# sczhou/ProPainter

Hardware: NVIDIA B200
Metric: inpainted frames/sec at 432x240x80f (higher is better)
Workload: dtype f32 (TF32 tensor-core products, fp32 accumulate)

## Files before the change

### include/propainter_b200.h

```cpp
#ifndef PROPAINTER_B200_H
#define PROPAINTER_B200_H
#include <stddef.h>
#include <stdint.h>
#include <cuda_runtime_api.h>

#ifdef __cplusplus
extern "C" {
#endif

#define PP_ABI_VERSION 2
int pp_abi_version(void);
const char* pp_error_string(int code);

int pp_corr_build(const float* fmap, int D, const int* idx1, const int* idx2, int n_pairs, float* lvl0, int h, int w,
                  cudaStream_t stream);
int pp_corr_pool_pyramid(float* const* levels, long planes, int h, int w, cudaStream_t stream);
int pp_corr_lookup(const float* const* levels, const float* coords, float* out, long n_pairs, int h, int w,
                   cudaStream_t stream);
int pp_corr_lookup_ldg(const float* const* levels, const float* coords, float* out, long n_pairs, int h, int w,
                       cudaStream_t stream);
int pp_convex_upsample(const float* mask, int ld_mask, float mask_scale, const float* flow_lr, float* out, int n,
                       int h, int w, cudaStream_t stream);

size_t pp_img_prop_scan_workspace_bytes(int t, int H, int W);
// ... 1 lines not shown
                     float* out_frames, float* out_masks, void* workspace, size_t ws_bytes, int t, int H, int W,
                     int nearest, cudaStream_t stream);
int pp_prop_cond(const float* cur, int ld_cur, const float* prop, int ld_prop, const float* fprop,
                 const float* fcheck, const float* mcur, float* cond, int ld_cond, float* bb, int ld_bb, int h, int w,
                 int C, int first, cudaStream_t stream);
size_t pp_deform_align_workspace_bytes(int H, int W);
int pp_deform_align(const float* x, int ld_x, const float* o, int ld_o, const float* o_bias, const float* flow, float max_res,
                    const float* w_packed, const float* bias, float* out, int ld_out, int H, int W, int Cin, int Cout,
                    void* workspace, size_t ws_bytes, cudaStream_t stream);
#define PP_CONV_MAX_SEG 4
typedef struct PPConvSeg { const float* x; int ld; int C; } PPConvSeg;
typedef struct PPConvParams {
  PPConvSeg seg[PP_CONV_MAX_SEG];
  int nseg;
  int n, H, W, KH, KW;
  const float* w_packed;
  int Cout;
  const float* bias;
  const float* pre; int ld_pre;
  const float* res; int ld_res;
  float* out; int ld_out;
  int act; float slope; int post_relu; int round_tf32;
  int bn, tile_w, tile_m;
} PPConvParams;
int pp_conv2d_umma(const PPConvParams* prm, cudaStream_t stream);
int pp_conv2d_umma_plan(const PPConvParams* prm, int* tile_h, int* tile_w, int* bn, int* ctas, int* smem_bytes);
int pp_deform_gather(const float* x, int ld_x, const float* x2, int ld_x2, const float* o, int ld_o, const float* o_bias,
                     const float* flow, float max_res, float* cols, int n, int H, int W, int Cin, cudaStream_t stream);
int pp_flow_warp_fbcheck(const float* feat, int ld_f, const float* fprop, const float* fcheck, float* warped, int ld_w,
                         float* aux, int ld_a, int n, int h, int w, int C, int round_tf32, cudaStream_t stream);

int pp_gen_prep(const float* flows_f, const float* flows_b, const float* masks_in, const float* masks_upd, float* dsf,
                float* dsb, float* pmask, int lt, int H, int W, cudaStream_t stream);
int pp_window_mask(const float* pmask, int lt, int h, int w, int fh, int fw, int nwh, int nww, int* flags,
                   cudaStream_t stream);

typedef struct PPAttnParams {
  const float* qkv;
  const float* pool;
  const int* key_tok;
  const int* flags;
  float* out;
  int ld_qkv, ld_pool, ld_out;
  int t, NT, WN, NKO, NP, C;
  int kf_start, kf_step, nkf;
  float scale_log2;
} PPAttnParams;
int pp_sparse_window_attn(const PPAttnParams* prm, int n_windows, cudaStream_t stream);
int pp_sparse_window_attn_mma(const PPAttnParams* prm, int n_windows, cudaStream_t stream);
// ... 50 lines not shown
```

### propainter_b200/_lib.py

```python
import ctypes
import os

_HERE = os.path.dirname(os.path.abspath(__file__))
LIB_PATH = os.environ.get("PROPAINTER_B200_LIB") or os.path.join(_HERE, "libpropainter_b200.so")

c_void_p, c_int, c_long, c_float, c_size_t = ctypes.c_void_p, ctypes.c_int, ctypes.c_long, ctypes.c_float, ctypes.c_size_t

PP_MAX_WINDOW = 32


class PPAttnParams(ctypes.Structure):
    _fields_ = [("qkv", c_void_p), ("pool", c_void_p), ("key_tok", c_void_p), ("flags", c_void_p), ("out", c_void_p),
                ("ld_qkv", c_int), ("ld_pool", c_int), ("ld_out", c_int),
                ("t", c_int), ("NT", c_int), ("WN", c_int), ("NKO", c_int), ("NP", c_int), ("C", c_int),
                ("kf_start", c_int), ("kf_step", c_int), ("nkf", c_int), ("scale_log2", c_float)]


PP_CONV_MAX_SEG = 4


class PPConvSeg(ctypes.Structure):
    _fields_ = [("x", c_void_p), ("ld", c_int), ("C", c_int)]


class PPConvParams(ctypes.Structure):
    _fields_ = [("seg", PPConvSeg * PP_CONV_MAX_SEG), ("nseg", c_int),
                ("n", c_int), ("H", c_int), ("W", c_int), ("KH", c_int), ("KW", c_int),
                ("w_packed", c_void_p), ("Cout", c_int), ("bias", c_void_p),
                ("pre", c_void_p), ("ld_pre", c_int), ("res", c_void_p), ("ld_res", c_int),
                ("out", c_void_p), ("ld_out", c_int),
                ("act", c_int), ("slope", c_float), ("post_relu", c_int), ("round_tf32", c_int),
                ("bn", c_int), ("tile_w", c_int), ("tile_m", c_int)]


class PPWindowIds(ctypes.Structure):
    _fields_ = [("n", c_int), ("frame", c_int * PP_MAX_WINDOW), ("first", c_int * PP_MAX_WINDOW)]


SIGNATURES = {
    "pp_abi_version": (c_int, []),
    "pp_error_string": (ctypes.c_char_p, [c_int]),
    "pp_corr_build": (c_int, [c_void_p, c_int, c_void_p, c_void_p, c_int, c_void_p, c_int, c_int, c_void_p]),
    "pp_corr_pool_pyramid": (c_int, [c_void_p, c_long, c_int, c_int, c_void_p]),
    "pp_corr_lookup": (c_int, [c_void_p, c_void_p, c_void_p, c_long, c_int, c_int, c_void_p]),
    "pp_corr_lookup_ldg": (c_int, [c_void_p, c_void_p, c_void_p, c_long, c_int, c_int, c_void_p]),
    "pp_convex_upsample": (c_int, [c_void_p, c_int, c_float, c_void_p, c_void_p, c_int, c_int, c_int, c_void_p]),
    "pp_img_prop_scan_workspace_bytes": (c_size_t, [c_int, c_int, c_int]),
    "pp_img_prop_scan": (c_int, [c_void_p, c_void_p, c_void_p, c_void_p, c_void_p, c_void_p, c_void_p, c_size_t, c_int,
                                 c_int, c_int, c_int, c_void_p]),
    "pp_prop_cond": (c_int, [c_void_p, c_int, c_void_p, c_int, c_void_p, c_void_p, c_void_p, c_void_p, c_int, c_void_p,
                             c_int, c_int, c_int, c_int, c_int, c_void_p]),
    "pp_deform_align_workspace_bytes": (c_size_t, [c_int, c_int]),
    "pp_deform_align": (c_int, [c_void_p, c_int, c_void_p, c_int, c_void_p, c_void_p, c_float, c_void_p, c_void_p, c_void_p,
                                c_int, c_int, c_int, c_int, c_int, c_void_p, c_size_t, c_void_p]),
    "pp_conv2d_umma": (c_int, [ctypes.POINTER(PPConvParams), c_void_p]),
    "pp_conv2d_umma_plan": (c_int, [ctypes.POINTER(PPConvParams)] + [c_void_p] * 5),
    "pp_deform_gather": (c_int, [c_void_p, c_int, c_void_p, c_int, c_void_p, c_int, c_void_p, c_void_p, c_float, c_void_p, c_int, c_int,
                                 c_int, c_int, c_void_p]),
    "pp_flow_warp_fbcheck": (c_int, [c_void_p, c_int, c_void_p, c_void_p, c_void_p, c_int, c_void_p, c_int, c_int, c_int, c_int, c_int,
                                     c_int, c_void_p]),
    "pp_gen_prep": (c_int, [c_void_p, c_void_p, c_void_p, c_void_p, c_void_p, c_void_p, c_void_p, c_int, c_int, c_int,
                            c_void_p]),
    "pp_window_mask": (c_int, [c_void_p, c_int, c_int, c_int, c_int, c_int, c_int, c_int, c_void_p, c_void_p]),
    "pp_sparse_window_attn": (c_int, [ctypes.POINTER(PPAttnParams), c_int, c_void_p]),
    "pp_sparse_window_attn_mma": (c_int, [ctypes.POINTER(PPAttnParams), c_int, c_void_p]),
    "pp_ffn_overlap_add_workspace_bytes": (c_size_t, [c_int, c_int, c_int, c_int]),
    "pp_ffn_overlap_add": (c_int, [c_void_p, c_int, c_void_p, c_int, c_int, c_int, c_int, c_int, c_void_p, c_size_t,
                                   c_void_p]),
    "pp_gru_gate": (c_int, [c_void_p, c_void_p, c_void_p, c_void_p, c_int, c_void_p, c_void_p, c_int, c_long, c_int, c_void_p]),
    "pp_gru_update": (c_int, [c_void_p, c_void_p, c_void_p, c_void_p, c_void_p, c_int, c_void_p, c_long, c_int, c_void_p]),
    "pp_raft_pack_motion": (c_int, [c_void_p, c_int, c_void_p, c_void_p, c_void_p, c_void_p, c_int, c_long, c_void_p]),
    "pp_bias_act": (c_int, [c_void_p, c_int, c_void_p, c_void_p, c_int, c_void_p, c_int, c_long, c_int, c_int, c_float, c_int,
                            c_void_p]),
    "pp_bias_act_pre": (c_int, [c_void_p, c_int, c_void_p, c_void_p, c_int, c_void_p, c_int, c_void_p, c_int, c_long, c_int, c_int, c_float,
                                c_int, c_void_p]),
    "pp_pool_depthwise": (c_int, [c_void_p, c_int, c_void_p, c_void_p, c_void_p, c_int, c_int, c_int, c_int, c_int, c_int, c_void_p]),
    "pp_add_layernorm": (c_int, [c_void_p, c_void_p, c_void_p, c_void_p, c_void_p, c_void_p, c_long, c_int, c_float, c_void_p]),
    "pp_instance_norm_workspace_bytes": (c_size_t, [c_int, c_long, c_int]),
    "pp_instance_norm": (c_int, [c_void_p, c_void_p, c_void_p, c_int, c_long, c_int, c_float, c_int, c_int, c_void_p, c_size_t,
# ... 41 lines not shown
```

### propainter_b200/csrc/conv_umma.cu

```cuda
#include <cuda.h>
#include <stdlib.h>
#include "pp_elem.cuh"
#include "pp_mma.cuh"
#include "pp_umma.cuh"
#include "../../include/propainter_b200.h"

#define CV_THREADS 192
#define CV_MAX_A_SLOTS 6
#define CV_MAX_B_SLOTS 8
#define CV_SMEM_BUDGET (216 * 1024)

struct alignas(64) CVParams {
  CUtensorMap tmA[PP_CONV_MAX_SEG];
  CUtensorMap tmB;
  int seg_blocks[PP_CONV_MAX_SEG];
  int seg_kblocks[PP_CONV_MAX_SEG];
  int nseg, nblk, kreal;
  int n, H, W, KH, KW, BH, BW, BN, M;
  int kgroup;
  int tiles_x, tiles_y;
  int na, nb;
  int ring_bytes;
  int a_copy_bytes;
  int Cout;
  const float* bias; const float* pre; const float* res; float* out;
  int ld_pre, ld_res, ld_out;
  int act, post_relu, round_tf32;
  float slope;
#ifdef CV_PROFILE
  long long* prof;
#endif
};

#ifdef CV_PROFILE
static long long* g_cv_prof = nullptr;
extern "C" void pp_conv_profile_buffer(long long* p) { g_cv_prof = p; }
#define CV_CLK() clock64()
#define CV_PROF(i, v) do { if (p.prof) p.prof[(long)(blockIdx.y * gridDim.x + blockIdx.x) * 16 + (i)] = (v); } while (0)
#else
#define CV_CLK() 0LL
#define CV_PROF(i, v) do { } while (0)
#endif

__device__ __forceinline__ void cv_expect_tx(uint32_t bar, uint32_t bytes) {
  asm volatile("mbarrier.arrive.expect_tx.shared::cta.b64 _, [%0], %1;" ::"r"(bar), "r"(bytes) : "memory");
}
__device__ __forceinline__ void cv_tma4(uint32_t dst, const CUtensorMap* tm, int c, int x, int y, int n, uint32_t bar) {
  asm volatile("cp.async.bulk.tensor.4d.shared::cluster.global.tile.mbarrier::complete_tx::bytes [%0], [%1, {%2, %3, %4, %5}], [%6];"
               ::"r"(dst), "l"(tm), "r"(c), "r"(x), "r"(y), "r"(n), "r"(bar) : "memory");
}
__device__ __forceinline__ void cv_tma2(uint32_t dst, const CUtensorMap* tm, int k, int n, uint32_t bar) {
  asm volatile("cp.async.bulk.tensor.2d.shared::cluster.global.tile.mbarrier::complete_tx::bytes [%0], [%1, {%2, %3}], [%4];"
               ::"r"(dst), "l"(tm), "r"(k), "r"(n), "r"(bar) : "memory");
}
__device__ __forceinline__ float cv_act(float v, int act, float slope) {
  switch (act) {
    case 1: return fmaxf(v, 0.f);
    case 2: return v > 0.f ? v : v * slope;
    case 3: return 1.0f / (1.0f + expf(-v));
    case 4: return tanhf(v);
    default: return v;
  }
}

__global__ void __launch_bounds__(CV_THREADS, 1) k_conv_umma(const __grid_constant__ CVParams p) {
  extern __shared__ __align__(1024) uint8_t cv_raw[];
  uint8_t* base = cv_raw + ((1024u - (ua_smem(cv_raw) & 1023u)) & 1023u);
  const int a_slot_bytes = p.KW * p.a_copy_bytes;
  const int b_tap_bytes = p.BN * 128, b_slot_bytes = p.KW * b_tap_bytes;
  uint8_t* sA = base;
  uint8_t* sB = sA + p.na * a_slot_bytes;
  uint8_t* tail = base + p.ring_bytes;
  unsigned long long* bars = reinterpret_cast<unsigned long long*>(tail);
  uint32_t* tmem_base_p = reinterpret_cast<uint32_t*>(tail + 40 * 8);
  const uint32_t b0 = ua_smem(bars);
  auto bar = [&](int i) { return b0 + 8u * (uint32_t)i; };
  const int tid = threadIdx.x, warp = tid >> 5, lane = tid & 31;
  const int tile = blockIdx.x, n0 = blockIdx.y * p.BN;
  const int tpi = p.tiles_x * p.tiles_y;
  const int img = tile / tpi, trem = tile - img * tpi;
  const int y0 = (trem / p.tiles_x) * p.BH, x0 = (trem % p.tiles_x) * p.BW;
  const int tmem_cols = p.BN < 32 ? 32 : p.BN;

  if (tid == 0) {
    for (int i = 0; i < p.na; ++i) { ua_bar_init(bar(i), 1); ua_bar_init(bar(8 + i), 1); }
    for (int i = 0; i < p.nb; ++i) { ua_bar_init(bar(16 + i), 1); ua_bar_init(bar(24 + i), 1); }
    ua_bar_init(bar(32), 1);
    asm volatile("fence.mbarrier_init.release.cluster;" ::: "memory");
  }
  if (warp == 5) {
    asm volatile("tcgen05.alloc.cta_group::1.sync.aligned.shared::cta.b32 [%0], %1;" ::"r"(ua_smem(tmem_base_p)), "r"(tmem_cols));
    asm volatile("tcgen05.relinquish_alloc_permit.cta_group::1.sync.aligned;");
  }
  asm volatile("tcgen05.fence::before_thread_sync;" ::: "memory");
  __syncthreads();
  asm volatile("tcgen05.fence::after_thread_sync;" ::: "memory");
  const uint32_t tD = *tmem_base_p;
  asm volatile("griddepcontrol.launch_dependents;");
  asm volatile("griddepcontrol.wait;" ::: "memory");

  if (warp == 4) {
    int seg = 0, cb = 0, kbase = 0;
    long long wa = 0, wb = 0, t1;
    (void)wa; (void)wb; (void)t1;
    CV_PROF(0, CV_CLK());
    for (int blk = 0; blk < p.nblk; ++blk) {
      const int sa = blk % p.na;
      t1 = CV_CLK();
      ua_bar_wait(bar(8 + sa), ((blk / p.na) & 1) ^ 1);
      wa += CV_CLK() - t1;
      if (ua_elect()) {
        cv_expect_tx(bar(sa), (uint32_t)a_slot_bytes);
        for (int dx = 0; dx < p.KW; ++dx)
          if (p.kgroup)
            cv_tma4(ua_smem(sA + sa * a_slot_bytes + dx * p.a_copy_bytes), &p.tmA[seg], (cb * p.KW + dx) * 32, x0, y0, img, bar(sa));
          else
            cv_tma4(ua_smem(sA + sa * a_slot_bytes + dx * p.a_copy_bytes), &p.tmA[seg], cb * 32, x0 + dx - p.KW / 2,
                    y0 - p.KH / 2, img, bar(sa));
      }
      __syncwarp();
      for (int dy = 0; dy < p.KH; ++dy) {
        const int ib = blk * p.KH + dy, sb = ib % p.nb;
        t1 = CV_CLK();
        ua_bar_wait(bar(24 + sb), ((ib / p.nb) & 1) ^ 1);
        wb += CV_CLK() - t1;
        if (ua_elect()) {
          cv_expect_tx(bar(16 + sb), (uint32_t)b_slot_bytes);
          for (int dx = 0; dx < p.KW; ++dx)
            cv_tma2(ua_smem(sB + sb * b_slot_bytes + dx * b_tap_bytes), &p.tmB,
                    (p.kgroup ? kbase + cb * p.KW + dx : ib * p.KW + dx) * 32, n0, bar(16 + sb));
        }
        __syncwarp();
      }
      if (++cb == p.seg_blocks[seg]) { cb = 0; kbase += p.seg_kblocks[seg]; ++seg; }
    }
    if (lane == 0) { CV_PROF(1, wa); CV_PROF(2, wb); CV_PROF(3, CV_CLK()); }
  } else if (warp == 5) {
    const uint32_t idesc = (1u << 4) | (2u << 7) | (2u << 10) | ((uint32_t)(p.BN >> 3) << 17) | ((uint32_t)(p.M >> 4) << 24);
    uint32_t acc = 0;
    long long wa = 0, wb = 0, t1, tfirst = 0;
    (void)wa; (void)wb; (void)t1; (void)tfirst;
    if (lane == 0) CV_PROF(4, CV_CLK());
    for (int blk = 0; blk < p.nblk; ++blk) {
      const int sa = blk % p.na;
      t1 = CV_CLK();
      ua_bar_wait(bar(sa), (blk / p.na) & 1);
      wa += CV_CLK() - t1;
      if (blk == 0) tfirst = CV_CLK();
      const uint64_t a_desc0 = ua_desc(ua_smem(sA + sa * a_slot_bytes));
      for (int dy = 0; dy < p.KH; ++dy) {
        const int ib = blk * p.KH + dy, sb = ib % p.nb;
        t1 = CV_CLK();
        ua_bar_wait(bar(16 + sb), (ib / p.nb) & 1);
        wb += CV_CLK() - t1;
        asm volatile("tcgen05.fence::after_thread_sync;" ::: "memory");
        const uint64_t b_desc0 = ua_desc(ua_smem(sB + sb * b_slot_bytes));
        if (ua_elect()) {
          uint64_t ad = a_desc0 + (uint64_t)((dy * p.BW * 128) >> 4), bd = b_desc0;
          for (int dx = 0; dx < p.KW; ++dx) {
#pragma unroll
            for (int ks = 0; ks < 4; ++ks) {
              ua_mma_ss(tD, ad + 2 * ks, bd + 2 * ks, idesc, acc);
              acc = 1;
            }
            ad += (uint64_t)(p.a_copy_bytes >> 4); bd += (uint64_t)(b_tap_bytes >> 4);
          }
          ua_commit(bar(24 + sb));
          if (dy == p.KH - 1) ua_commit(bar(8 + sa));
          if (dy == p.KH - 1 && blk == p.nblk - 1) ua_commit(bar(32));
        }
        acc = 1;
        __syncwarp();
      }
    }
    if (lane == 0) { CV_PROF(5, wa); CV_PROF(6, wb); CV_PROF(7, tfirst); CV_PROF(8, CV_CLK()); }
  } else {
    const uint32_t lane_off = (uint32_t)(warp * 32) << 16;
    const int rsub = lane >> 3, c4 = lane & 7;
    const float* __restrict__ bias = p.bias;
    const int act = p.act, post_relu = p.post_relu, round_tf32 = p.round_tf32;
    const float slope = p.slope;
    const int rpw = p.M >> 2, bw_shift = p.BW == 16 ? 4 : 3;
    const float* prow[8]; const float* rrow[8]; float* orow[8];
    unsigned okmask = 0;
#pragma unroll
    for (int i = 0; i < 8; ++i) {
      const int rl = 4 * i + rsub, r = warp * rpw + rl;
      const int y = y0 + (r >> bw_shift), x = x0 + (r & (p.BW - 1));
      const bool ok = rl < rpw && y < p.H && x < p.W;
      const long pix = ok ? ((long)img * p.H + y) * p.W + x : 0;
      okmask |= ok ? (1u << i) : 0u;
      orow[i] = p.out + pix * p.ld_out + n0 + 4 * c4;
      prow[i] = p.pre ? p.pre + pix * p.ld_pre + n0 + 4 * c4 : nullptr;
      rrow[i] = p.res ? p.res + pix * p.ld_res + n0 + 4 * c4 : nullptr;
      asm volatile("" : "+l"(orow[i]), "+l"(prow[i]), "+l"(rrow[i]));
    }
    const bool has_pre = p.pre != nullptr, has_res = p.res != nullptr;
    const int nchunk = p.BN >> 5;
    float* stgw = reinterpret_cast<float*>(sA) + warp * nchunk * (32 * 36);
    ua_bar_wait(bar(32), 0);
    if (tid == 0) CV_PROF(9, CV_CLK());
    asm volatile("tcgen05.fence::after_thread_sync;" ::: "memory");
    for (int ch = 0; ch < nchunk; ++ch) {
      uint32_t v[32];
      UA_LD32(tD + ch * 32 + lane_off, v);
      asm volatile("tcgen05.wait::ld.sync.aligned;" ::: "memory");
      float* stg = stgw + ch * (32 * 36);
#pragma unroll
      for (int j = 0; j < 8; ++j)
        *reinterpret_cast<float4*>(stg + lane * 36 + 4 * j) =
            make_float4(__uint_as_float(v[4 * j]), __uint_as_float(v[4 * j + 1]), __uint_as_float(v[4 * j + 2]), __uint_as_float(v[4 * j + 3]));
    }
    __syncwarp();
    if (tid == 0) CV_PROF(12, CV_CLK());
    for (int ch = 0; ch < nchunk; ++ch) {
      const int n = n0 + ch * 32 + 4 * c4;
      const bool n_in = n < p.Cout;
      const float* stg = stgw + ch * (32 * 36);
      float4 bv = make_float4(0.f, 0.f, 0.f, 0.f), pv[8], rv[8];
      if (bias && n_in) bv = __ldg(reinterpret_cast<const float4*>(bias + n));
      const unsigned on = n_in ? okmask : 0u;
#pragma unroll
      for (int i = 0; i < 8; ++i) {
        pv[i] = (has_pre && ((on >> i) & 1)) ? *reinterpret_cast<const float4*>(prow[i] + ch * 32) : make_float4(0.f, 0.f, 0.f, 0.f);
        rv[i] = (has_res && ((on >> i) & 1)) ? *reinterpret_cast<const float4*>(rrow[i] + ch * 32) : make_float4(0.f, 0.f, 0.f, 0.f);
      }
      auto finish = [&](auto actf) {
        float4 a[8];
#pragma unroll
        for (int i = 0; i < 8; ++i) a[i] = *reinterpret_cast<const float4*>(stg + (4 * i + rsub) * 36 + 4 * c4);
#pragma unroll
        for (int i = 0; i < 8; ++i) {
          a[i].x = actf(a[i].x + (bv.x + pv[i].x)) + rv[i].x; a[i].y = actf(a[i].y + (bv.y + pv[i].y)) + rv[i].y;
          a[i].z = actf(a[i].z + (bv.z + pv[i].z)) + rv[i].z; a[i].w = actf(a[i].w + (bv.w + pv[i].w)) + rv[i].w;
          if (post_relu) { a[i].x = fmaxf(a[i].x, 0.f); a[i].y = fmaxf(a[i].y, 0.f); a[i].z = fmaxf(a[i].z, 0.f); a[i].w = fmaxf(a[i].w, 0.f); }
          if (round_tf32) {
            a[i].x = __uint_as_float(pp_tf32(a[i].x)); a[i].y = __uint_as_float(pp_tf32(a[i].y));
            a[i].z = __uint_as_float(pp_tf32(a[i].z)); a[i].w = __uint_as_float(pp_tf32(a[i].w));
          }
        }
#pragma unroll
        for (int i = 0; i < 8; ++i)
          if ((on >> i) & 1) *reinterpret_cast<float4*>(orow[i] + ch * 32) = a[i];
      };
      if (act == 0) finish([](float v) { return v; });
      else if (act == 1) finish([](float v) { return fmaxf(v, 0.f); });
      else if (act == 2) finish([slope](float v) { return v > 0.f ? v : v * slope; });
      else if (act == 3) finish([](float v) { return 1.0f / (1.0f + expf(-v)); });
      else finish([](float v) { return tanhf(v); });
    }
    if (tid == 0) CV_PROF(14, CV_CLK());
  }
  asm volatile("tcgen05.fence::before_thread_sync;" ::: "memory");
  __syncthreads();
  if (tid == 0) CV_PROF(10, CV_CLK());
  if (warp == 5) asm volatile("tcgen05.dealloc.cta_group::1.sync.aligned.b32 %0, %1;" ::"r"(tD), "r"(tmem_cols));
}

static bool cv_pdl_enabled() {
  static int on = -1;
  if (on < 0) { const char* e = getenv("PP_PDL"); on = (e && e[0] == '0') ? 0 : 1; }
  return on != 0;
}
template <typename... KArgs, typename... Args>
static cudaError_t cv_launch(void (*kernel)(KArgs...), dim3 grid, dim3 block, size_t smem, cudaStream_t stream, Args... args) {
  cudaLaunchConfig_t cfg = {};
  cfg.gridDim = grid; cfg.blockDim = block; cfg.dynamicSmemBytes = smem; cfg.stream = stream;
  cudaLaunchAttribute attr[1];
  attr[0].id = cudaLaunchAttributeProgrammaticStreamSerialization;
  attr[0].val.programmaticStreamSerializationAllowed = 1;
  cfg.attrs = attr; cfg.numAttrs = cv_pdl_enabled() ? 1 : 0;
  return cudaLaunchKernelEx(&cfg, kernel, KArgs(args)...);
}

typedef CUresult (*PFN_cvEncodeTiled)(CUtensorMap*, CUtensorMapDataType, cuuint32_t, void*, const cuuint64_t*, const cuuint64_t*,
                                      const cuuint32_t*, const cuuint32_t*, CUtensorMapInterleave, CUtensorMapSwizzle,
                                      CUtensorMapL2promotion, CUtensorMapFloatOOBfill);
static PFN_cvEncodeTiled cv_encoder() {
  static PFN_cvEncodeTiled cached = nullptr;
  if (cached) return cached;
  void* fn = nullptr;
  cudaDriverEntryPointQueryResult qres;
  if (cudaGetDriverEntryPoint("cuTensorMapEncodeTiled", &fn, cudaEnableDefault, &qres) != cudaSuccess ||
      qres != cudaDriverEntryPointSuccess)
    return nullptr;
  cached = (PFN_cvEncodeTiled)fn;
  return cached;
}

static int cv_plan(const PPConvParams* q, CVParams* p, int* smem_bytes) {
  if (q->nseg < 1 || q->nseg > PP_CONV_MAX_SEG || q->n < 1 || q->H < 1 || q->W < 1) return PP_ERR_SHAPE;
  if (q->KH < 1 || q->KW < 1 || q->KH > 7 || q->KW > 7 || !(q->KH & 1) || !(q->KW & 1)) return PP_ERR_SHAPE;
  if (q->Cout < 4 || q->Cout % 4) return PP_ERR_SHAPE;
  int nblk = 0, kblocks = 0;
  for (int s = 0; s < q->nseg; ++s) {
// ... 7 lines not shown
  for (int s = 0; s < q->nseg; ++s) {
    p->seg_blocks[s] = kv ? (p->seg_kblocks[s] + kv - 1) / kv : p->seg_kblocks[s];
    nblk += p->seg_blocks[s];
  }
  if (q->ld_out % 4 || ((uintptr_t)q->out & 15) || ((uintptr_t)q->w_packed & 15)) return PP_ERR_ALIGN;
  if (q->bias && ((uintptr_t)q->bias & 15)) return PP_ERR_ALIGN;
  if (q->pre && (q->ld_pre % 4 || ((uintptr_t)q->pre & 15))) return PP_ERR_ALIGN;
  if (q->res && (q->ld_res % 4 || ((uintptr_t)q->res & 15))) return PP_ERR_ALIGN;
  p->nseg = q->nseg; p->nblk = nblk;
  p->n = q->n; p->H = q->H; p->W = q->W; p->KH = q->KH; p->KW = kv ? kv : q->KW;
  p->kreal = kblocks;
  int bw = q->tile_w;
  if (bw != 8 && bw != 16) {
    const int mm = q->tile_m == 64 ? 64 : 128;
    const long a8 = (long)((q->W + 7) / 8) * ((q->H + mm / 8 - 1) / (mm / 8)), a16 = (long)((q->W + 15) / 16) * ((q->H + mm / 16 - 1) / (mm / 16));
    bw = a16 < a8 ? 16 : 8;
  }
  const int M = q->tile_m == 64 ? 64 : 128;
  p->M = M;
  p->BW = bw; p->BH = M / bw;
  p->tiles_x = (q->W + p->BW - 1) / p->BW; p->tiles_y = (q->H + p->BH - 1) / p->BH;
  const long tiles = (long)p->tiles_x * p->tiles_y * q->n;
  if (tiles > 0x7fffffffL) return PP_ERR_SHAPE;
  int bn = q->bn;
  if (bn != 32 && bn != 64 && bn != 128) {
    long best = -1;
    for (int cand = 128; cand >= 32; cand >>= 1) {
      const long ctas = tiles * ((q->Cout + cand - 1) / cand), waves = (ctas + PP_NUM_SMS - 1) / PP_NUM_SMS;
      const long cost = waves * (850 + 23 * cand / 10);
      if (best < 0 || cost < best) { best = cost; bn = cand; }
    }
  }
  p->BN = bn;
  p->a_copy_bytes = (p->BH + p->KH - 1) * p->BW * 128;
  const int a_slot = p->KW * p->a_copy_bytes, b_slot = p->KW * bn * 128;
  int na = (q->KH * q->KW == 1 && !p->kgroup) ? 4 : 2;
  if (na > nblk) na = nblk;
  if (na * a_slot + b_slot > CV_SMEM_BUDGET) na = 1;
  if (na * a_slot + b_slot > CV_SMEM_BUDGET) return PP_ERR_SHAPE;
  int nb = (CV_SMEM_BUDGET - na * a_slot) / b_slot;
  if (nb > CV_MAX_B_SLOTS) nb = CV_MAX_B_SLOTS;
  if (nb > nblk * q->KH) nb = nblk * q->KH;
  while (na < CV_MAX_A_SLOTS && na < nblk && (na + 1) * a_slot + nb * b_slot <= CV_SMEM_BUDGET) ++na;
  p->na = na; p->nb = nb;
  p->ring_bytes = na * a_slot + nb * b_slot;
  if (p->ring_bytes < 4 * (bn / 32) * 32 * 36 * 4) p->ring_bytes = 4 * (bn / 32) * 32 * 36 * 4;
  *smem_bytes = p->ring_bytes + 512 + 1024;
  p->Cout = q->Cout;
  p->bias = q->bias; p->pre = q->pre; p->res = q->res; p->out = q->out;
  p->ld_pre = q->ld_pre; p->ld_res = q->ld_res; p->ld_out = q->ld_out;
  p->act = q->act; p->post_relu = q->post_relu; p->round_tf32 = q->round_tf32; p->slope = q->slope;
  return PP_OK;
}

extern "C" int pp_conv2d_umma_plan(const PPConvParams* q, int* tile_h, int* tile_w, int* bn, int* ctas, int* smem_bytes) {
  CVParams p;
  int smem = 0;
  const int rc = cv_plan(q, &p, &smem);
  if (rc != PP_OK) return rc;
  if (tile_h) *tile_h = p.BH;
  if (tile_w) *tile_w = p.BW;
  if (bn) *bn = p.BN;
  if (ctas) *ctas = p.tiles_x * p.tiles_y * p.n * ((p.Cout + p.BN - 1) / p.BN);
  if (smem_bytes) *smem_bytes = smem;
  return PP_OK;
}

extern "C" int pp_conv2d_umma(const PPConvParams* q, cudaStream_t stream) {
  CVParams p;
  int smem = 0;
  int rc = cv_plan(q, &p, &smem);
  if (rc != PP_OK) return rc;
  PFN_cvEncodeTiled enc = cv_encoder();
  if (!enc) return PP_ERR_LAUNCH;
  for (int s = 0; s < q->nseg; ++s) {
    const cuuint64_t ld = (cuuint64_t)q->seg[s].ld;
    cuuint64_t dims[4] = {(cuuint64_t)q->seg[s].C, (cuuint64_t)q->W, (cuuint64_t)q->H, (cuuint64_t)q->n};
    cuuint64_t strides[3] = {ld * 4, ld * 4 * (cuuint64_t)q->W, ld * 4 * (cuuint64_t)q->W * (cuuint64_t)q->H};
    cuuint32_t box[4] = {32, (cuuint32_t)p.BW, (cuuint32_t)(p.BH + p.KH - 1), 1};
    cuuint32_t estr[4] = {1, 1, 1, 1};
    if (enc(&p.tmA[s], CU_TENSOR_MAP_DATA_TYPE_FLOAT32, 4, (void*)q->seg[s].x, dims, strides, box, estr, CU_TENSOR_MAP_INTERLEAVE_NONE,
            CU_TENSOR_MAP_SWIZZLE_128B, CU_TENSOR_MAP_L2_PROMOTION_L2_128B, CU_TENSOR_MAP_FLOAT_OOB_FILL_NONE) != CUDA_SUCCESS)
      return PP_ERR_LAUNCH;
  }
  {
    const cuuint64_t ktot = (cuuint64_t)p.kreal * q->KH * q->KW * 32;
    cuuint64_t dims[2] = {ktot, (cuuint64_t)q->Cout};
    cuuint64_t strides[1] = {ktot * 4};
    cuuint32_t box[2] = {32, (cuuint32_t)p.BN};
    cuuint32_t estr[2] = {1, 1};
    if (enc(&p.tmB, CU_TENSOR_MAP_DATA_TYPE_FLOAT32, 2, (void*)q->w_packed, dims, strides, box, estr, CU_TENSOR_MAP_INTERLEAVE_NONE,
            CU_TENSOR_MAP_SWIZZLE_128B, CU_TENSOR_MAP_L2_PROMOTION_L2_256B, CU_TENSOR_MAP_FLOAT_OOB_FILL_NONE) != CUDA_SUCCESS)
      return PP_ERR_LAUNCH;
  }
  if (cudaFuncSetAttribute(k_conv_umma, cudaFuncAttributeMaxDynamicSharedMemorySize, CV_SMEM_BUDGET + 2048) != cudaSuccess)
    return PP_ERR_LAUNCH;
#ifdef CV_PROFILE
  p.prof = g_cv_prof;
#endif
  dim3 grid((unsigned)(p.tiles_x * p.tiles_y * p.n), (unsigned)((p.Cout + p.BN - 1) / p.BN));
  if (cv_launch(k_conv_umma, grid, dim3(CV_THREADS), (size_t)smem, stream, p) != cudaSuccess) return PP_ERR_LAUNCH;
  return cudaPeekAtLastError() == cudaSuccess ? PP_OK : PP_ERR_LAUNCH;
}

template <int CPL>
__global__ void __launch_bounds__(256) k_deform_gather(const float* __restrict__ x, int ld_x, const float* __restrict__ x2, int ld_x2,
    const float* __restrict__ o, int ld_o,
    const float* __restrict__ obias, const float* __restrict__ flow, float max_res, float* __restrict__ cols, long npix, int H, int W) {
  asm volatile("griddepcontrol.launch_dependents;");
  asm volatile("griddepcontrol.wait;" ::: "memory");
  const long pix = (long)blockIdx.x * 8 + (threadIdx.x >> 5);
  if (pix >= npix) return;
  const int lane = threadIdx.x & 31, g = lane >> 1, half = lane & 1;
  const long HW = (long)H * W, img = pix / HW, pim = pix - img * HW;
  const int y = (int)(pim / W), xx = (int)(pim - (long)y * W);
  const float* op = o + pix * ld_o;
  float2 off[9]; float ml[9];
#pragma unroll
  for (int k = 0; k < 9; ++k) { off[k] = *reinterpret_cast<const float2*>(op + g * 18 + 2 * k); ml[k] = op[288 + g * 9 + k]; }
  float fy = 0.f, fx = 0.f;
  if (flow) { fx = flow[2 * pix]; fy = flow[2 * pix + 1]; }
  if (obias) {
#pragma unroll
    for (int k = 0; k < 9; ++k) { off[k].x += obias[g * 18 + 2 * k]; off[k].y += obias[g * 18 + 2 * k + 1]; ml[k] += obias[288 + g * 9 + k]; }
// ... 63 lines not shown
```

### propainter_b200/ops.py

```python
import ctypes
import math

import torch

from . import _lib
from ._lib import PPAttnParams, PPConvParams, PPWindowIds, check

LOG2E = 1.4426950408889634

LAUNCHES = 0


def _count(n):
    global LAUNCHES
    LAUNCHES += n


def _stream():
    return ctypes.c_void_p(torch.cuda.current_stream().cuda_stream)


def _p(t, dtype=torch.float32):
    if t is None:
        return None
# ... 113 lines not shown
def pack_conv_weight(weight, seg_channels=None):
    Cout, Cin, KH, KW = weight.shape
    seg_channels = [Cin] if seg_channels is None else list(seg_channels)
    if sum(seg_channels) != Cin:
        raise RuntimeError("pack_conv_weight: segments do not add up to Cin")
    blocks, c0 = [], 0
    for C in seg_channels:
        for b in range(0, C, 32):
            cw = min(32, C - b)
            blk = weight.new_zeros(Cout, KH, KW, 32)
            blk[..., :cw] = weight[:, c0 + b:c0 + b + cw].permute(0, 2, 3, 1)
            blocks.append(blk.reshape(Cout, KH * KW * 32))
        c0 += C
    return tf32_round(torch.cat(blocks, 1).contiguous())


def _pm4(t):
    if t.dim() != 4:
        raise RuntimeError("expected [n,H,W,C]")
    return _pm(t)


def conv_umma(segs, w_packed, KH, KW, Cout, bias=None, act="none", slope=0.0, pre=None, res=None, post_relu=False, out=None,
              round_tf32=False, bn=0, tile_w=0, tile_m=0):
    n, H, W, _ = segs[0].shape
    if out is None:
        out = torch.empty(n, H, W, Cout, device=segs[0].device, dtype=torch.float32)
    prm = PPConvParams()
    prm.nseg = len(segs)
    kblocks = 0
    for i, sgm in enumerate(segs):
        if tuple(sgm.shape[:3]) != (n, H, W):
            raise RuntimeError("conv_umma: segment shape mismatch")
        ptr, ld = _pm4(sgm)
        prm.seg[i].x, prm.seg[i].ld, prm.seg[i].C = ptr.value, ld, sgm.shape[-1]
        kblocks += (sgm.shape[-1] + 31) // 32
    if tuple(w_packed.shape) != (Cout, kblocks * KH * KW * 32):
        raise RuntimeError(f"conv_umma: packed weight {tuple(w_packed.shape)} does not match {(Cout, kblocks * KH * KW * 32)}")
    prm.n, prm.H, prm.W, prm.KH, prm.KW = n, H, W, KH, KW
    prm.w_packed, prm.Cout = _p(_dense(w_packed)).value, Cout
    prm.bias = _p(bias).value if bias is not None else None
    for name, t in (("pre", pre), ("res", res), ("out", out)):
        if t is None:
            setattr(prm, name, None)
            setattr(prm, "ld_" + name, 0)
            continue
        if tuple(t.shape) != (n, H, W, Cout):
            raise RuntimeError(f"conv_umma: {name} shape {tuple(t.shape)} != {(n, H, W, Cout)}")
        ptr, ld = _pm4(t)
        setattr(prm, name, ptr.value)
        setattr(prm, "ld_" + name, ld)
    prm.act, prm.slope, prm.post_relu, prm.round_tf32 = ACT[act], float(slope), int(bool(post_relu)), int(bool(round_tf32))
    prm.bn, prm.tile_w, prm.tile_m = int(bn), int(tile_w), int(tile_m)
    check(_lib.lib().pp_conv2d_umma(ctypes.byref(prm), _stream()), "pp_conv2d_umma")
    _count(1)
    return out


def deform_gather(x, o, flow, max_res, cols=None, o_bias=None, x2=None):
    n, H, W, Cin = x.shape
    xp, ldx = _pm4(x)
    x2p, ldx2 = (None, 0)
    if x2 is not None:
        if x2.shape != x.shape:
            raise RuntimeError("deform_gather: x2 must have the shape of x")
        x2p, ldx2 = _pm4(x2)
        Cin *= 2
    op, ldo = _pm4(o)
    if cols is None:
        cols = torch.empty(n, H, W, 9 * Cin, device=x.device, dtype=torch.float32)
    check(_lib.lib().pp_deform_gather(xp, ldx, x2p, ldx2, op, ldo, _p(o_bias), _p(_dense(flow)) if flow is not None else None,
                                      float(max_res), _p(_dense(cols)), n, H, W, Cin, _stream()), "pp_deform_gather")
    _count(1)
    return cols


# ... 279 lines not shown
```

Baseline: 357.0.

## Add cluster-based split-K to UMMA conv with DSMEM reduction

Adds a split-K mode to the tcgen05 implicit-GEMM conv kernel: each output tile is split across a thread-block cluster of up to 8 CTAs, each handling a slice of the K (channel-block x kernel-row) units. Partial accumulators are staged in shared memory and reduced by reading peer CTAs' smem through distributed shared memory, with cluster barriers around the epilogue. The planner now jointly picks BN and split factor using a cost model that considers cluster occupancy. The goal is more CTAs for small-resolution convs (e.g. 30x54 recurrent flow-completion steps) that otherwise underfill the SMs. The cost is extra cluster syncs and DSMEM traffic, and cluster scheduling limits.

```diff
diff --git a/include/propainter_b200.h b/include/propainter_b200.h
--- a/include/propainter_b200.h
+++ b/include/propainter_b200.h
@@ -47,9 +47,10 @@
   float* out; int ld_out;
   int act; float slope; int post_relu; int round_tf32;
   int bn, tile_w, tile_m;
+  int ksplit;
 } PPConvParams;
 int pp_conv2d_umma(const PPConvParams* prm, cudaStream_t stream);
-int pp_conv2d_umma_plan(const PPConvParams* prm, int* tile_h, int* tile_w, int* bn, int* ctas, int* smem_bytes);
+int pp_conv2d_umma_plan(const PPConvParams* prm, int* tile_h, int* tile_w, int* bn, int* ctas, int* smem_bytes, int* ksplit);
 int pp_deform_gather(const float* x, int ld_x, const float* x2, int ld_x2, const float* o, int ld_o, const float* o_bias,
                      const float* flow, float max_res, float* cols, int n, int H, int W, int Cin, cudaStream_t stream);
 int pp_flow_warp_fbcheck(const float* feat, int ld_f, const float* fprop, const float* fcheck, float* warped, int ld_w,
diff --git a/profiles/scan_conv_times.py b/profiles/scan_conv_times.py
--- /dev/null
+++ b/profiles/scan_conv_times.py
@@ -0,0 +1,110 @@
+import argparse
+import ctypes
+import json
+import os
+import statistics
+import sys
+
+import torch
+
+ROOT = os.path.dirname(os.path.dirname(os.path.abspath(__file__)))
+sys.path.insert(0, ROOT)
+
+
+def plan_of(ops, segs, Cout, KH, KW, ksplit):
+    from propainter_b200 import _lib
+    prm = _lib.PPConvParams()
+    prm.nseg = len(segs)
+    for i, s in enumerate(segs):
+        ptr, ld = ops._pm4(s)
+        prm.seg[i].x, prm.seg[i].ld, prm.seg[i].C = ptr.value, ld, s.shape[-1]
+    prm.n, prm.H, prm.W = segs[0].shape[:3]
+    prm.KH, prm.KW, prm.Cout, prm.ksplit = KH, KW, Cout, ksplit
+    prm.w_packed, prm.out, prm.ld_out = 1 << 20, 1 << 20, Cout
+    v = [ctypes.c_int() for _ in range(6)]
+    _lib.check(_lib.lib().pp_conv2d_umma_plan(ctypes.byref(prm), *(ctypes.byref(x) for x in v)), "pp_conv2d_umma_plan")
+    return {"bn": v[2].value, "ctas": v[3].value, "ksplit": v[5].value}
+
+
+def main():
+    ap = argparse.ArgumentParser()
+    ap.add_argument("--reps", type=int, default=50)
+    ap.add_argument("--out", default=None)
+    a = ap.parse_args()
+    import __graft_entry__
+    __graft_entry__.build()
+    from propainter_b200 import ops
+    assert torch.cuda.is_available(), "needs a CUDA device"
+    dev = "cuda"
+    torch.backends.cuda.matmul.allow_tf32 = False
+    flush = torch.empty(256 << 20, dtype=torch.uint8, device=dev)
+    gen = torch.Generator().manual_seed(0)
+
+    def t(fn):
+        for _ in range(3):
+            fn()
+        ts = []
+        for _ in range(a.reps):
+            flush.zero_()
+            e0, e1 = torch.cuda.Event(enable_timing=True), torch.cuda.Event(enable_timing=True)
+            e0.record()
+            fn()
+            e1.record()
+            e1.synchronize()
+            ts.append(e0.elapsed_time(e1) * 1e3)
+        return statistics.median(ts)
+
+    def rnd(*shape):
+        return ops.tf32_round(torch.randn(*shape, generator=gen)).to(dev)
+
+    rows, sums = [], {}
+    for scan, (h, w), cin_d, max_res in (("rfc", (30, 54), 256, 5.0), ("gen", (60, 108), 128, 3.0)):
+        C = 128
+        s1, s2, x = rnd(1, h, w, C), rnd(1, h, w, C), rnd(1, h, w, C)
+        pre, res = rnd(1, h, w, C), rnd(1, h, w, C)
+        out, o = torch.empty(1, h, w, C, device=dev), torch.empty(1, h, w, 432, device=dev)
+        off0_segs = [s1, s2] if scan == "rfc" else [x]
+        convs = [
+            ("conv_offset.0", off0_segs, C, 3, 3, dict(pre=pre, act="leaky", slope=0.1, round_tf32=True, out=out), 1),
+            ("conv_offset.2/.4", [x], C, 3, 3, dict(bias=pre[0, 0, 0], act="leaky", slope=0.1, round_tf32=True, out=out), 2),
+            ("conv_offset.6", [x], 432, 3, 3, dict(bias=torch.zeros(432, device=dev), out=o), 1),
+            ("backbone.0", [x], C, 3, 3, dict(pre=pre, act="leaky", slope=0.1, round_tf32=True, out=out), 1),
+            ("backbone.2", [x], C, 3, 3, dict(bias=pre[0, 0, 0], res=res, out=out), 1),
+        ]
+        cols = torch.empty(1, h, w, 9 * cin_d, device=dev)
+        convs.append(("deform GEMM 1x1", [cols], C, 1, 1, dict(bias=pre[0, 0, 0], out=out), 1))
+        xg = rnd(1, h, w, cin_d)
+        og = (torch.randn(1, h, w, 432, generator=gen) * 1.5).to(dev)
+        fl = (torch.randn(1, h, w, 2, generator=gen) * 2).to(dev) if scan == "gen" else None
+        if scan == "rfc":
+            xa, xb = xg[..., :128].contiguous(), xg[..., 128:].contiguous()
+            gather = lambda: ops.deform_gather(xa, og, None, max_res, cols, x2=xb)
+        else:
+            gather = lambda: ops.deform_gather(xg, og, fl, max_res, cols)
+        gather()
+        us = t(gather)
+        rows.append({"scan": scan, "kernel": "k_deform_gather", "us": round(us, 2)})
+        sums[(scan, 1)] = sums[(scan, 0)] = us
+        for name, segs, Cout, KH, KW, kw, per_step in convs:
+            Cin = sum(s.shape[-1] for s in segs)
+            wp = ops.pack_conv_weight(torch.randn(Cout, Cin, KH, KW, generator=gen) / (Cin * KH * KW) ** 0.5,
+                                      [s.shape[-1] for s in segs]).to(dev)
+            for ks in (1, 0):
+                us = t(lambda: ops.conv_umma(segs, wp, KH, KW, Cout, ksplit=ks, **kw))
+                flop = 2.0 * h * w * Cin * KH * KW * Cout
+                rows.append({"scan": scan, "kernel": f"k_conv_umma {name}", "ksplit": "auto" if ks == 0 else 1,
+                             "plan": plan_of(ops, segs, Cout, KH, KW, ks), "us": round(us, 2), "tflops": round(flop / us / 1e6, 1)})
+                sums[(scan, ks)] += per_step * us
+    for r in rows:
+        print(json.dumps(r))
+    summary = {f"{scan}_step_us_{'auto' if ks == 0 else 'ksplit1'}": round(v, 1) for (scan, ks), v in sums.items()}
+    summary["device"] = torch.cuda.get_device_name()
+    print(json.dumps(summary))
+    if a.out:
+        os.makedirs(a.out, exist_ok=True)
+        with open(os.path.join(a.out, "scan_conv_times.json"), "w") as f:
+            json.dump({"rows": rows, "summary": summary}, f, indent=1)
+
+
+if __name__ == "__main__":
+    main()
diff --git a/propainter_b200/_lib.py b/propainter_b200/_lib.py
--- a/propainter_b200/_lib.py
+++ b/propainter_b200/_lib.py
@@ -30,7 +30,7 @@
                 ("pre", c_void_p), ("ld_pre", c_int), ("res", c_void_p), ("ld_res", c_int),
                 ("out", c_void_p), ("ld_out", c_int),
                 ("act", c_int), ("slope", c_float), ("post_relu", c_int), ("round_tf32", c_int),
-                ("bn", c_int), ("tile_w", c_int), ("tile_m", c_int)]
+                ("bn", c_int), ("tile_w", c_int), ("tile_m", c_int), ("ksplit", c_int)]
 
 
 class PPWindowIds(ctypes.Structure):
@@ -54,7 +54,7 @@
     "pp_deform_align": (c_int, [c_void_p, c_int, c_void_p, c_int, c_void_p, c_void_p, c_float, c_void_p, c_void_p, c_void_p,
                                 c_int, c_int, c_int, c_int, c_int, c_void_p, c_size_t, c_void_p]),
     "pp_conv2d_umma": (c_int, [ctypes.POINTER(PPConvParams), c_void_p]),
-    "pp_conv2d_umma_plan": (c_int, [ctypes.POINTER(PPConvParams)] + [c_void_p] * 5),
+    "pp_conv2d_umma_plan": (c_int, [ctypes.POINTER(PPConvParams)] + [c_void_p] * 6),
     "pp_deform_gather": (c_int, [c_void_p, c_int, c_void_p, c_int, c_void_p, c_int, c_void_p, c_void_p, c_float, c_void_p, c_int, c_int,
                                  c_int, c_int, c_void_p]),
     "pp_flow_warp_fbcheck": (c_int, [c_void_p, c_int, c_void_p, c_void_p, c_void_p, c_int, c_void_p, c_int, c_int, c_int, c_int, c_int,
diff --git a/propainter_b200/csrc/conv_umma.cu b/propainter_b200/csrc/conv_umma.cu
--- a/propainter_b200/csrc/conv_umma.cu
+++ b/propainter_b200/csrc/conv_umma.cu
@@ -23,6 +23,7 @@
   int ring_bytes;
   int a_copy_bytes;
   int Cout;
+  int ksplit;
   const float* bias; const float* pre; const float* res; float* out;
   int ld_pre, ld_res, ld_out;
   int act, post_relu, round_tf32;
@@ -52,6 +53,16 @@
 __device__ __forceinline__ void cv_tma2(uint32_t dst, const CUtensorMap* tm, int k, int n, uint32_t bar) {
   asm volatile("cp.async.bulk.tensor.2d.shared::cluster.global.tile.mbarrier::complete_tx::bytes [%0], [%1, {%2, %3}], [%4];"
                ::"r"(dst), "l"(tm), "r"(k), "r"(n), "r"(bar) : "memory");
+}
+__device__ __forceinline__ void cv_cluster_sync() {
+  asm volatile("barrier.cluster.arrive.release;\n\tbarrier.cluster.wait.acquire;" ::: "memory");
+}
+__device__ __forceinline__ float4 cv_ld_dsmem(uint32_t saddr, int rank) {
+  uint32_t ra;
+  float4 v;
+  asm volatile("mapa.shared::cluster.u32 %0, %1, %2;" : "=r"(ra) : "r"(saddr), "r"(rank));
+  asm volatile("ld.shared::cluster.v4.f32 {%0, %1, %2, %3}, [%4];" : "=f"(v.x), "=f"(v.y), "=f"(v.z), "=f"(v.w) : "r"(ra) : "memory");
+  return v;
 }
 __device__ __forceinline__ float cv_act(float v, int act, float slope) {
   switch (act) {
@@ -76,7 +87,10 @@
   const uint32_t b0 = ua_smem(bars);
   auto bar = [&](int i) { return b0 + 8u * (uint32_t)i; };
   const int tid = threadIdx.x, warp = tid >> 5, lane = tid & 31;
-  const int tile = blockIdx.x, n0 = blockIdx.y * p.BN;
+  const int S = p.ksplit, rank = blockIdx.x % S;
+  const int tile = blockIdx.x / S, n0 = blockIdx.y * p.BN;
+  const int units = p.nblk * p.KH, u0 = rank * units / S, u1 = (rank + 1) * units / S;
+  const int blk_lo = u0 / p.KH, blk_hi = (u1 - 1) / p.KH;
   const int tpi = p.tiles_x * p.tiles_y;
   const int img = tile / tpi, trem = tile - img * tpi;
   const int y0 = (trem / p.tiles_x) * p.BH, x0 = (trem % p.tiles_x) * p.BW;
@@ -104,10 +118,15 @@
     long long wa = 0, wb = 0, t1;
     (void)wa; (void)wb; (void)t1;
     CV_PROF(0, CV_CLK());
-    for (int blk = 0; blk < p.nblk; ++blk) {
-      const int sa = blk % p.na;
+    int la = 0, lb = 0;
+    for (int blk = 0; blk <= blk_hi; ++blk) {
+      if (blk < blk_lo) {
+        if (++cb == p.seg_blocks[seg]) { cb = 0; kbase += p.seg_kblocks[seg]; ++seg; }
+        continue;
+      }
+      const int sa = la % p.na;
       t1 = CV_CLK();
-      ua_bar_wait(bar(8 + sa), ((blk / p.na) & 1) ^ 1);
+      ua_bar_wait(bar(8 + sa), ((la / p.na) & 1) ^ 1);
       wa += CV_CLK() - t1;
       if (ua_elect()) {
         cv_expect_tx(bar(sa), (uint32_t)a_slot_bytes);
@@ -119,10 +138,11 @@
                     y0 - p.KH / 2, img, bar(sa));
       }
       __syncwarp();
-      for (int dy = 0; dy < p.KH; ++dy) {
-        const int ib = blk * p.KH + dy, sb = ib % p.nb;
+      const int dy_lo = max(u0 - blk * p.KH, 0), dy_hi = min(u1 - blk * p.KH, p.KH);
+      for (int dy = dy_lo; dy < dy_hi; ++dy, ++lb) {
+        const int ib = blk * p.KH + dy, sb = lb % p.nb;
         t1 = CV_CLK();
-        ua_bar_wait(bar(24 + sb), ((ib / p.nb) & 1) ^ 1);
+        ua_bar_wait(bar(24 + sb), ((lb / p.nb) & 1) ^ 1);
         wb += CV_CLK() - t1;
         if (ua_elect()) {
           cv_expect_tx(bar(16 + sb), (uint32_t)b_slot_bytes);
@@ -132,26 +152,30 @@
         }
         __syncwarp();
       }
+      ++la;
       if (++cb == p.seg_blocks[seg]) { cb = 0; kbase += p.seg_kblocks[seg]; ++seg; }
     }
     if (lane == 0) { CV_PROF(1, wa); CV_PROF(2, wb); CV_PROF(3, CV_CLK()); }
+    if (S > 1) cv_cluster_sync();
   } else if (warp == 5) {
     const uint32_t idesc = (1u << 4) | (2u << 7) | (2u << 10) | ((uint32_t)(p.BN >> 3) << 17) | ((uint32_t)(p.M >> 4) << 24);
     uint32_t acc = 0;
     long long wa = 0, wb = 0, t1, tfirst = 0;
     (void)wa; (void)wb; (void)t1; (void)tfirst;
     if (lane == 0) CV_PROF(4, CV_CLK());
-    for (int blk = 0; blk < p.nblk; ++blk) {
-      const int sa = blk % p.na;
+    int la = 0, lb = 0;
+    for (int blk = blk_lo; blk <= blk_hi; ++blk, ++la) {
+      const int sa = la % p.na;
       t1 = CV_CLK();
-      ua_bar_wait(bar(sa), (blk / p.na) & 1);
+      ua_bar_wait(bar(sa), (la / p.na) & 1);
       wa += CV_CLK() - t1;
-      if (blk == 0) tfirst = CV_CLK();
+      if (la == 0) tfirst = CV_CLK();
       const uint64_t a_desc0 = ua_desc(ua_smem(sA + sa * a_slot_bytes));
-      for (int dy = 0; dy < p.KH; ++dy) {
-        const int ib = blk * p.KH + dy, sb = ib % p.nb;
+      const int dy_lo = max(u0 - blk * p.KH, 0), dy_hi = min(u1 - blk * p.KH, p.KH);
+      for (int dy = dy_lo; dy < dy_hi; ++dy, ++lb) {
+        const int sb = lb % p.nb;
         t1 = CV_CLK();
-        ua_bar_wait(bar(16 + sb), (ib / p.nb) & 1);
+        ua_bar_wait(bar(16 + sb), (lb / p.nb) & 1);
         wb += CV_CLK() - t1;
         asm volatile("tcgen05.fence::after_thread_sync;" ::: "memory");
         const uint64_t b_desc0 = ua_desc(ua_smem(sB + sb * b_slot_bytes));
@@ -166,14 +190,15 @@
             ad += (uint64_t)(p.a_copy_bytes >> 4); bd += (uint64_t)(b_tap_bytes >> 4);
           }
           ua_commit(bar(24 + sb));
-          if (dy == p.KH - 1) ua_commit(bar(8 + sa));
-          if (dy == p.KH - 1 && blk == p.nblk - 1) ua_commit(bar(32));
+          if (dy == dy_hi - 1) ua_commit(bar(8 + sa));
+          if (dy == dy_hi - 1 && blk == blk_hi) ua_commit(bar(32));
         }
         acc = 1;
         __syncwarp();
       }
     }
     if (lane == 0) { CV_PROF(5, wa); CV_PROF(6, wb); CV_PROF(7, tfirst); CV_PROF(8, CV_CLK()); }
+    if (S > 1) cv_cluster_sync();
   } else {
     const uint32_t lane_off = (uint32_t)(warp * 32) << 16;
     const int rsub = lane >> 3, c4 = lane & 7;
@@ -181,13 +206,21 @@
     const int act = p.act, post_relu = p.post_relu, round_tf32 = p.round_tf32;
     const float slope = p.slope;
     const int rpw = p.M >> 2, bw_shift = p.BW == 16 ? 4 : 3;
+    const int nchunk = p.BN >> 5;
+    int rfirst = warp * rpw, rcount = rpw, ch0 = 0, chstep = 1;
+    if (S > 1) {
+      const int R = p.M / S, G = R > 32 ? 2 : 1;
+      rfirst = rank * R + (warp % G) * 32; rcount = min(32, R - (warp % G) * 32); ch0 = warp / G; chstep = 4 / G;
+    }
     const float* prow[8]; const float* rrow[8]; float* orow[8];
+    int sofs[8];
     unsigned okmask = 0;
 #pragma unroll
     for (int i = 0; i < 8; ++i) {
-      const int rl = 4 * i + rsub, r = warp * rpw + rl;
+      const int rl = 4 * i + rsub, r = rfirst + rl;
       const int y = y0 + (r >> bw_shift), x = x0 + (r & (p.BW - 1));
-      const bool ok = rl < rpw && y < p.H && x < p.W;
+      const bool ok = rl < rcount && y < p.H && x < p.W;
+      sofs[i] = rl < rcount ? (r / rpw) * nchunk * (32 * 36) + (r % rpw) * 36 + 4 * c4 : 0;
       const long pix = ok ? ((long)img * p.H + y) * p.W + x : 0;
       okmask |= ok ? (1u << i) : 0u;
       orow[i] = p.out + pix * p.ld_out + n0 + 4 * c4;
@@ -196,7 +229,6 @@
       asm volatile("" : "+l"(orow[i]), "+l"(prow[i]), "+l"(rrow[i]));
     }
     const bool has_pre = p.pre != nullptr, has_res = p.res != nullptr;
-    const int nchunk = p.BN >> 5;
     float* stgw = reinterpret_cast<float*>(sA) + warp * nchunk * (32 * 36);
     ua_bar_wait(bar(32), 0);
     if (tid == 0) CV_PROF(9, CV_CLK());
@@ -212,11 +244,13 @@
             make_float4(__uint_as_float(v[4 * j]), __uint_as_float(v[4 * j + 1]), __uint_as_float(v[4 * j + 2]), __uint_as_float(v[4 * j + 3]));
     }
     __syncwarp();
+    if (S > 1) cv_cluster_sync();
     if (tid == 0) CV_PROF(12, CV_CLK());
-    for (int ch = 0; ch < nchunk; ++ch) {
+    const float* stg0 = reinterpret_cast<const float*>(sA);
+    for (int ch = ch0; ch < nchunk; ch += chstep) {
       const int n = n0 + ch * 32 + 4 * c4;
       const bool n_in = n < p.Cout;
-      const float* stg = stgw + ch * (32 * 36);
+      const float* stg = stg0 + ch * (32 * 36);
       float4 bv = make_float4(0.f, 0.f, 0.f, 0.f), pv[8], rv[8];
       if (bias && n_in) bv = __ldg(reinterpret_cast<const float4*>(bias + n));
       const unsigned on = n_in ? okmask : 0u;
@@ -227,8 +261,23 @@
       }
       auto finish = [&](auto actf) {
         float4 a[8];
-#pragma unroll
-        for (int i = 0; i < 8; ++i) a[i] = *reinterpret_cast<const float4*>(stg + (4 * i + rsub) * 36 + 4 * c4);
+        if (S == 1) {
+#pragma unroll
+          for (int i = 0; i < 8; ++i) a[i] = *reinterpret_cast<const float4*>(stg + sofs[i]);
+        } else {
+#pragma unroll
+          for (int i = 0; i < 8; ++i) {
+            a[i] = make_float4(0.f, 0.f, 0.f, 0.f);
+            if ((on >> i) & 1) {
+              const uint32_t sa = ua_smem(stg + sofs[i]);
+              a[i] = cv_ld_dsmem(sa, 0);
+              for (int s = 1; s < S; ++s) {
+                const float4 v = cv_ld_dsmem(sa, s);
+                a[i].x += v.x; a[i].y += v.y; a[i].z += v.z; a[i].w += v.w;
+              }
+            }
+          }
+        }
 #pragma unroll
         for (int i = 0; i < 8; ++i) {
           a[i].x = actf(a[i].x + (bv.x + pv[i].x)) + rv[i].x; a[i].y = actf(a[i].y + (bv.y + pv[i].y)) + rv[i].y;
@@ -251,6 +300,7 @@
     }
     if (tid == 0) CV_PROF(14, CV_CLK());
   }
+  if (S > 1) cv_cluster_sync();
   asm volatile("tcgen05.fence::before_thread_sync;" ::: "memory");
   __syncthreads();
   if (tid == 0) CV_PROF(10, CV_CLK());
@@ -263,14 +313,47 @@
   return on != 0;
 }
 template <typename... KArgs, typename... Args>
-static cudaError_t cv_launch(void (*kernel)(KArgs...), dim3 grid, dim3 block, size_t smem, cudaStream_t stream, Args... args) {
+static cudaError_t cv_launch_cluster(void (*kernel)(KArgs...), dim3 grid, dim3 block, size_t smem, cudaStream_t stream, int cluster,
+                                     Args... args) {
   cudaLaunchConfig_t cfg = {};
   cfg.gridDim = grid; cfg.blockDim = block; cfg.dynamicSmemBytes = smem; cfg.stream = stream;
-  cudaLaunchAttribute attr[1];
-  attr[0].id = cudaLaunchAttributeProgrammaticStreamSerialization;
-  attr[0].val.programmaticStreamSerializationAllowed = 1;
-  cfg.attrs = attr; cfg.numAttrs = cv_pdl_enabled() ? 1 : 0;
+  cudaLaunchAttribute attr[2];
+  int na = 0;
+  if (cv_pdl_enabled()) {
+    attr[na].id = cudaLaunchAttributeProgrammaticStreamSerialization;
+    attr[na++].val.programmaticStreamSerializationAllowed = 1;
+  }
+  if (cluster > 1) {
+    attr[na].id = cudaLaunchAttributeClusterDimension;
+    attr[na].val.clusterDim.x = (unsigned)cluster; attr[na].val.clusterDim.y = 1; attr[na++].val.clusterDim.z = 1;
+  }
+  cfg.attrs = attr; cfg.numAttrs = (unsigned)na;
   return cudaLaunchKernelEx(&cfg, kernel, KArgs(args)...);
+}
+template <typename... KArgs, typename... Args>
+static cudaError_t cv_launch(void (*kernel)(KArgs...), dim3 grid, dim3 block, size_t smem, cudaStream_t stream, Args... args) {
+  return cv_launch_cluster(kernel, grid, block, smem, stream, 1, args...);
+}
+
+static int cv_cluster_capacity(int s) {
+  static int cached[9] = {0};
+  if (s <= 1) return PP_NUM_SMS;
+  if (!cached[s]) {
+    int n = 0;
+    if (cudaFuncSetAttribute(k_conv_umma, cudaFuncAttributeMaxDynamicSharedMemorySize, CV_SMEM_BUDGET + 2048) == cudaSuccess) {
+      cudaLaunchConfig_t cfg = {};
+      cfg.gridDim = dim3((unsigned)(s * PP_NUM_SMS)); cfg.blockDim = dim3(CV_THREADS); cfg.dynamicSmemBytes = CV_SMEM_BUDGET + 2048;
+      cudaLaunchAttribute attr[1];
+      attr[0].id = cudaLaunchAttributeClusterDimension;
+      attr[0].val.clusterDim.x = (unsigned)s; attr[0].val.clusterDim.y = 1; attr[0].val.clusterDim.z = 1;
+      cfg.attrs = attr; cfg.numAttrs = 1;
+      if (cudaOccupancyMaxActiveClusters(&n, (void*)k_conv_umma, &cfg) != cudaSuccess) { n = 0; cudaGetLastError(); }
+    } else {
+      cudaGetLastError();
+    }
+    cached[s] = n > 0 ? n * s : (PP_NUM_SMS / s) * s;
+  }
+  return cached[s];
 }
 
 typedef CUresult (*PFN_cvEncodeTiled)(CUtensorMap*, CUtensorMapDataType, cuuint32_t, void*, const cuuint64_t*, const cuuint64_t*,
@@ -324,16 +407,26 @@
   p->tiles_x = (q->W + p->BW - 1) / p->BW; p->tiles_y = (q->H + p->BH - 1) / p->BH;
   const long tiles = (long)p->tiles_x * p->tiles_y * q->n;
   if (tiles > 0x7fffffffL) return PP_ERR_SHAPE;
-  int bn = q->bn;
-  if (bn != 32 && bn != 64 && bn != 128) {
+  const int units = nblk * q->KH, mma_per_unit = p->KW * 4;
+  int bn = q->bn, ks = q->ksplit;
+  if (ks < 0 || ks > 8 || (ks & (ks - 1)) || ks > units) return PP_ERR_SHAPE;
+  {
+    const bool bn_free = bn != 32 && bn != 64 && bn != 128;
     long best = -1;
-    for (int cand = 128; cand >= 32; cand >>= 1) {
-      const long ctas = tiles * ((q->Cout + cand - 1) / cand), waves = (ctas + PP_NUM_SMS - 1) / PP_NUM_SMS;
-      const long cost = waves * (850 + 23 * cand / 10);
-      if (best < 0 || cost < best) { best = cost; bn = cand; }
-    }
-  }
+    int best_bn = bn, best_s = 1;
+    for (int s = ks ? ks : 1; s <= (ks ? ks : 8) && s <= units; s <<= 1)
+      for (int cand = bn_free ? 128 : bn; cand >= (bn_free ? 32 : bn); cand >>= 1) {
+        const long ctas = tiles * ((q->Cout + cand - 1) / cand) * s, cap = cv_cluster_capacity(s);
+        const long waves = (ctas + cap - 1) / cap;
+        const long nmma = (long)((units + s - 1) / s) * mma_per_unit;
+        const long cost = waves * (4000 + nmma * (42 + cand / 2) + (s > 1 ? 4000 + (long)M * cand / 8 : 0));
+        if (best < 0 || cost < best) { best = cost; best_bn = cand; best_s = s; }
+      }
+    bn = best_bn; ks = best_s;
+  }
+  if (tiles * ks > 0x7fffffffL) return PP_ERR_SHAPE;
   p->BN = bn;
+  p->ksplit = ks;
   p->a_copy_bytes = (p->BH + p->KH - 1) * p->BW * 128;
   const int a_slot = p->KW * p->a_copy_bytes, b_slot = p->KW * bn * 128;
   int na = (q->KH * q->KW == 1 && !p->kgroup) ? 4 : 2;
@@ -355,7 +448,7 @@
   return PP_OK;
 }
 
-extern "C" int pp_conv2d_umma_plan(const PPConvParams* q, int* tile_h, int* tile_w, int* bn, int* ctas, int* smem_bytes) {
+extern "C" int pp_conv2d_umma_plan(const PPConvParams* q, int* tile_h, int* tile_w, int* bn, int* ctas, int* smem_bytes, int* ksplit) {
   CVParams p;
   int smem = 0;
   const int rc = cv_plan(q, &p, &smem);
@@ -363,8 +456,9 @@
   if (tile_h) *tile_h = p.BH;
   if (tile_w) *tile_w = p.BW;
   if (bn) *bn = p.BN;
-  if (ctas) *ctas = p.tiles_x * p.tiles_y * p.n * ((p.Cout + p.BN - 1) / p.BN);
+  if (ctas) *ctas = p.tiles_x * p.tiles_y * p.n * ((p.Cout + p.BN - 1) / p.BN) * p.ksplit;
   if (smem_bytes) *smem_bytes = smem;
+  if (ksplit) *ksplit = p.ksplit;
   return PP_OK;
 }
 
@@ -400,8 +494,8 @@
 #ifdef CV_PROFILE
   p.prof = g_cv_prof;
 #endif
-  dim3 grid((unsigned)(p.tiles_x * p.tiles_y * p.n), (unsigned)((p.Cout + p.BN - 1) / p.BN));
-  if (cv_launch(k_conv_umma, grid, dim3(CV_THREADS), (size_t)smem, stream, p) != cudaSuccess) return PP_ERR_LAUNCH;
+  dim3 grid((unsigned)(p.tiles_x * p.tiles_y * p.n * p.ksplit), (unsigned)((p.Cout + p.BN - 1) / p.BN));
+  if (cv_launch_cluster(k_conv_umma, grid, dim3(CV_THREADS), (size_t)smem, stream, p.ksplit, p) != cudaSuccess) return PP_ERR_LAUNCH;
   return cudaPeekAtLastError() == cudaSuccess ? PP_OK : PP_ERR_LAUNCH;
 }
 
diff --git a/propainter_b200/ops.py b/propainter_b200/ops.py
--- a/propainter_b200/ops.py
+++ b/propainter_b200/ops.py
@@ -159,7 +159,7 @@
 
 
 def conv_umma(segs, w_packed, KH, KW, Cout, bias=None, act="none", slope=0.0, pre=None, res=None, post_relu=False, out=None,
-              round_tf32=False, bn=0, tile_w=0, tile_m=0):
+              round_tf32=False, bn=0, tile_w=0, tile_m=0, ksplit=0):
     n, H, W, _ = segs[0].shape
     if out is None:
         out = torch.empty(n, H, W, Cout, device=segs[0].device, dtype=torch.float32)
@@ -188,7 +188,7 @@
         setattr(prm, name, ptr.value)
         setattr(prm, "ld_" + name, ld)
     prm.act, prm.slope, prm.post_relu, prm.round_tf32 = ACT[act], float(slope), int(bool(post_relu)), int(bool(round_tf32))
-    prm.bn, prm.tile_w, prm.tile_m = int(bn), int(tile_w), int(tile_m)
+    prm.bn, prm.tile_w, prm.tile_m, prm.ksplit = int(bn), int(tile_w), int(tile_m), int(ksplit)
     check(_lib.lib().pp_conv2d_umma(ctypes.byref(prm), _stream()), "pp_conv2d_umma")
     _count(1)
     return out
```

Result: no change. 354.6 (median of 6 runs) (-0.7%).
